# vfmatzkin/ct-unet

Hardware: AMD Instinct MI355X
Metric: voxels/sec fwd+bwd, 128^3 fp32 patch (higher is better)
Workload: dtype f32; 1 GPU; UNet() default (1 in, 2 out, i_size 8, 4 blocks), 128^3 patch, batch 1 per GPU, train step = fwd + Dice/CE loss + bwd + grad all-reduce + Adam(amsgrad); patch=128, per_gpu_batch=1, parallelism=dp1, launch=hipgraph

## Files before the change

### ct-unet_amd/csrc/conv3d.hip

```cpp
#include "common.h"
#include "pack.h"
#include "bn_tail.h"

#ifndef CTU_K3S_OCC
#define CTU_K3S_OCC 2
#endif
#ifndef CTU_K3S_ALL
#define CTU_K3S_ALL 1
#endif
#ifndef CTU_WG_OCC
#define CTU_WG_OCC 2
#endif
#ifndef CTU_WG_BLOCKS
#define CTU_WG_BLOCKS 512
#endif

namespace {

typedef float gv2f __attribute__((ext_vector_type(2)));

struct ConvP {
    const float* in;
    const float* in_scale;
    const float* in_shift;
// ... 1056 lines not shown
    const bool a_ok = (ci0 + quad * 4) < p.cin_p, g_ok = (co0 + quad * 4) < p.cout_p;
    const bool has_xf = p.in_scale != nullptr;
    float4 sc = make_float4(1.f, 1.f, 1.f, 1.f), sh = make_float4(0.f, 0.f, 0.f, 0.f);
    if (has_xf && a_ok) {
        sc = *reinterpret_cast<const float4*>(p.in_scale + ci0 + quad * 4);
        sh = *reinterpret_cast<const float4*>(p.in_shift + ci0 + quad * 4);
    }

    for (int tile = blockIdx.x; tile < p.ntiles; tile += gridDim.x) {
        int bx = tile;
        const int tx = bx % p.tiles_w; bx /= p.tiles_w;
        const int ty = bx % p.tiles_h; bx /= p.tiles_h;
        const int tz = bx % p.tiles_d; bx /= p.tiles_d;
        const int n_img = bx;
        const int d0 = tz * TD, h0 = ty * TH, w0 = tx * TW;
        __syncthreads();
        constexpr int SB = 8;
        const size_t img = (size_t)n_img * p.D * p.H * p.W;
        for (int it0 = tid; it0 < HV * 4; it0 += SB * 256) {
            f32x4 vv[SB];
            unsigned okm = 0;
#pragma unroll
            for (int q = 0; q < SB; ++q) {
                const int it = it0 + q * 256;
                const int v = (it < HV * 4 ? it : it0) >> 2;
                const int pw = v % HW, t2 = v / HW, ph = t2 % HH, pd = t2 / HH;
                const int gd = d0 + pd + kd0 - PAD, gh = h0 + ph - PAD, gw = w0 + pw - PAD;
                const bool ok = a_ok && (unsigned)gd < (unsigned)p.D && (unsigned)gh < (unsigned)p.H && (unsigned)gw < (unsigned)p.W;
                okm |= ok ? (1u << q) : 0u;
                const size_t off = ok ? ((size_t)(gd * p.H + gh) * p.W + gw) * p.in_cs + ci0 + quad * 4 : (size_t)0;
                vv[q] = *reinterpret_cast<const f32x4*>(p.in + img * p.in_cs + off);
            }
#pragma unroll
            for (int q = 0; q < SB; ++q) {
                const int it = it0 + q * 256;
                if (it < HV * 4) {
                    float4 val = make_float4(vv[q][0], vv[q][1], vv[q][2], vv[q][3]);
                    if (has_xf) val = xform4(val, sc, sh, p.in_relu);
                    if (!((okm >> q) & 1u)) val = make_float4(0.f, 0.f, 0.f, 0.f);
                    *reinterpret_cast<float4*>(&sA[(it >> 2) * 16 + quad * 4]) = val;
                }
            }
        }
        for (int it0 = tid; it0 < NVOX * 4; it0 += SB * 256) {
            f32x4 vv[SB];
            unsigned okm = 0;
#pragma unroll
            for (int q = 0; q < SB; ++q) {
                const int it = it0 + q * 256;
                const int v = (it < NVOX * 4 ? it : it0) >> 2;
                const int tw = v % TW, th = (v / TW) % TH, td = v / (TW * TH);
                const int gd = d0 + td, gh = h0 + th, gw = w0 + tw;
                const bool ok = g_ok && gd < p.D && gh < p.H && gw < p.W;
                okm |= ok ? (1u << q) : 0u;
                const size_t off = ok ? ((size_t)(gd * p.H + gh) * p.W + gw) * p.g_cs + co0 + quad * 4 : (size_t)0;
                vv[q] = *reinterpret_cast<const f32x4*>(p.g + img * p.g_cs + off);
            }
#pragma unroll
            for (int q = 0; q < SB; ++q) {
                const int it = it0 + q * 256;
                if (it < NVOX * 4)
                    *reinterpret_cast<f32x4*>(&sG[(it >> 2) * 16 + quad * 4]) = ((okm >> q) & 1u) ? vv[q] : f32x4{0.f, 0.f, 0.f, 0.f};
            }
        }
        __syncthreads();
#pragma unroll 2
        for (int ks = 0; ks < KPW; ++ks) {
            const int vt = (wave * KPW + ks) * 4 + kq;
            const int tw = vt % TW, th = (vt / TW) % TH, td = vt / (TW * TH);
            const float b = sG[vt * 16 + i];
            const int ab = ((td * HH + th) * HW + tw) * 16 + i;
#pragma unroll
            for (int t = 0; t < BT; ++t) {
                const int kd = t / (KS * KS), kh = (t / KS) % KS, kw = t % KS;
                const float a = sA[ab + ((kd * HH + kh) * HW + kw) * 16];
                acc[t] = __builtin_amdgcn_mfma_f32_16x16x4f32(a, b, acc[t], 0, 0, 0);
            }
        }
    }
    constexpr int RT = (HV * 16 / 1024) < 8 ? (HV * 16 / 1024) : 8;
    static_assert(RT >= 1 && 4 * RT * 256 <= HV * 16, "reduction scratch must fit in sA");
    const size_t slab = (size_t)(blockIdx.z * gridDim.y + blockIdx.y) * gridDim.x + blockIdx.x;
    float* dst = p.ws + slab * (BT * 256);
    for (int t0 = 0; t0 < BT; t0 += RT) {
        __syncthreads();
#pragma unroll
        for (int t = 0; t < BT; ++t)
            if (t >= t0 && t < t0 + RT) {
#pragma unroll
                for (int r = 0; r < 4; ++r) sA[(wave * RT + (t - t0)) * 256 + (kq * 4 + r) * 16 + i] = acc[t][r];
            }
        __syncthreads();
        const int nt = (BT - t0) < RT ? (BT - t0) : RT;
        for (int e = tid; e < nt * 256; e += 256)
            dst[t0 * 256 + e] = (sA[e] + sA[RT * 256 + e]) + (sA[2 * RT * 256 + e] + sA[3 * RT * 256 + e]);
    }
}

template <int KS, int KDS>
__global__ __launch_bounds__(1024) void conv3d_wgrad_reduce_kernel(const float* __restrict__ ws, float* __restrict__ dw,
                                                                  int Co, int Ci, const int32_t* __restrict__ pmap,
                                                                  int cin_p, int n_ci_t, int gx) {
    constexpr int TAPS = KS * KS * KS, BT = KDS * KS * KS;
    __shared__ float red[RPARTS][64];
    const int e = threadIdx.x & 63, part = threadIdx.x >> 6;
    const int el = blockIdx.x * 64 + e;
    const int pz = blockIdx.y;
    float s = 0.f;
    if (el < BT * 256) {
        const float* src = ws + (size_t)pz * gx * (BT * 256) + el;
        for (int k = part; k < gx; k += RPARTS) s += src[(size_t)k * (BT * 256)];
    }
    red[part][e] = s;
    __syncthreads();
    if (part == 0 && el < BT * 256) {
        const float tot = red_total(red, e);
        const int n_pairs = gridDim.y / (TAPS / BT);
        const int z = pz / n_pairs, pair = pz % n_pairs;
        const int cit = pair % n_ci_t, cot = pair / n_ci_t;
        const int tl = el >> 8, i = (el >> 4) & 15, j = el & 15;
        const int cip = cit * 16 + i, co = cot * 16 + j;
        const int ci = (cip < cin_p) ? (pmap ? pmap[cip] : (cip < Ci ? cip : -1)) : -1;
        if (ci >= 0 && co < Co) dw[((size_t)co * Ci + ci) * TAPS + z * BT + tl] = tot;
    }
}

inline bool use_k3s(int k, int W, int cin_p, int cout_p) { return k == 3 && W >= 16 && (CTU_K3S_ALL || cin_p == 8 || cout_p == 8); }

inline int wgrad_gx(int ntiles, int pairs_z) {
    int gx = CTU_WG_BLOCKS / pairs_z;
    if (gx < 1) gx = 1;
    if (gx > ntiles) gx = ntiles;
    return gx;
}


template <int SM, int SN, int UP = 0, bool LZ = false>
__global__ __launch_bounds__(256, CTU_K3S_OCC) void conv3d_wgrad_k3s_kernel(WgP p, int tiles_per_block) {
    static_assert(!UP || (SM == 1 && SN == 1), "the fused up-convolution uses the full 16 x 16 channel tile");
    constexpr int TD = 4, TH = 4, TW = (SM == 2 && SN == 2) ? 16 : 8, HD = 6, HH = 6, HW = TW + 2, HV = HD * HH * HW;
    constexpr int KPR = TW / 4, NKS = TH * KPR;
    constexpr int CM = 16 / SM, CN = 16 / SN;
    constexpr int GW = TW + (SN - 1), GV = TD * TH * GW;
    constexpr int QN = (SM == 2 && SN == 2) ? 1 : ((SM == 1 && SN == 1) ? 3 : 2);
    constexpr int NMF = UP == 2 ? 12 : (UP ? 8 : 9 * QN);
    constexpr int AQ = CM / 4, GQ = CN / 4;
    constexpr int AITEMS = HV * AQ, AITER = (AITEMS + 255) / 256;
    constexpr int GITEMS = GV * GQ, GITER = (GITEMS + 255) / 256;

    constexpr int SAF = AITER * 256 * 4, SGF = GITER * 256 * 4;
    static_assert(SAF >= HV * CM && SGF >= GV * CN, "stage size");
    __shared__ __attribute__((aligned(16))) float sA[2 * SAF];
    __shared__ __attribute__((aligned(16))) float sG[2 * SGF];

    const int tid = threadIdx.x, lane = tid & 63, wave = tid >> 6;
    const int i = lane & 15, kq = lane >> 4;
    const int cig = blockIdx.y % p.n_ci_t, cog = UP ? (blockIdx.y / p.n_ci_t) % p.n_co_t : blockIdx.y / p.n_ci_t;
    const int par = UP ? blockIdx.y / (p.n_ci_t * p.n_co_t) : 0;
    const int pz = UP == 2 ? (par >> 1) & 1 : (par >> 2) & 1, py = UP == 2 ? par & 1 : (par >> 1) & 1, px = UP == 2 ? 0 : par & 1;
    const int gH = UP ? 2 * p.H : p.H, gW = UP ? 2 * p.W : p.W, gs = UP ? 2 : 1;
    const int ci0 = cig * CM, co0 = cog * CN;
    const bool has_xf = p.in_scale != nullptr;

    f32x4 acc[NMF];
#pragma unroll
    for (int t = 0; t < NMF; ++t) acc[t] = f32x4{0.f, 0.f, 0.f, 0.f};

    const int aq = tid % AQ, gq = tid % GQ;
    const bool a_ok = (ci0 + aq * 4) < p.cin_p, g_ok = (co0 + gq * 4) < p.cout_p;
    float4 sc = make_float4(1.f, 1.f, 1.f, 1.f), sh = make_float4(0.f, 0.f, 0.f, 0.f);
    if (has_xf && a_ok) {
        sc = *reinterpret_cast<const float4*>(p.in_scale + ci0 + aq * 4);
        sh = *reinterpret_cast<const float4*>(p.in_shift + ci0 + aq * 4);
    }
    const int xf_relu = has_xf ? p.in_relu : 0;
    const int boff = (SN == 2) ? ((i < 8) ? i : i - 16) : i;

    int tile = blockIdx.x * tiles_per_block;
    const int tile_end = min(p.ntiles, tile + tiles_per_block);
    float4 va[AITER], vg[GITER];
    float4 vy[LZ ? GITER : 1];
    float4 l_sc = make_float4(0.f, 0.f, 0.f, 0.f), l_sh = l_sc, l_k0 = l_sc, l_A = l_sc, l_B = l_sc;
    if constexpr (LZ) {
        const int lzc = (co0 + ((UP && !g_ok) ? 0 : gq * 4)) % p.lz_cp;
        l_sc = *reinterpret_cast<const float4*>(p.lz_scale + lzc);
        l_sh = *reinterpret_cast<const float4*>(p.lz_shift + lzc);
        l_k0 = *reinterpret_cast<const float4*>(p.lz_coef + lzc);
        l_A = *reinterpret_cast<const float4*>(p.lz_coef + 3 * p.lz_cp + lzc);
        l_B = *reinterpret_cast<const float4*>(p.lz_coef + 4 * p.lz_cp + lzc);
    }
    const long long lz_ydelta = LZ ? reinterpret_cast<const char*>(p.lz_y) - reinterpret_cast<const char*>(p.g) : 0;
    const long long lz_odelta = LZ ? reinterpret_cast<const char*>(p.lz_out) - reinterpret_cast<const char*>(p.g) : 0;

    unsigned aoff[AITER], goff[GITER];
    constexpr int FPW = 5;
    unsigned fw[(AITER + FPW - 1) / FPW], gw0 = 0;
#pragma unroll
    for (int q = 0; q < (AITER + FPW - 1) / FPW; ++q) fw[q] = 0;
#pragma unroll
    for (int it = 0; it < AITER; ++it) {
        const int e = tid + it * 256, v = (e < AITEMS) ? e / AQ : 0;
        const int pw = v % HW, t2 = v / HW, ph = t2 % HH, pd = t2 / HH;
        aoff[it] = (unsigned)(((pd * p.H + ph) * p.W + pw) * p.in_cs + ci0 + aq * 4) * 4u;
        const unsigned face = (pd == 0 ? 1u : 0u) | (pd == HD - 1 ? 2u : 0u) | (ph == 0 ? 4u : 0u) | (ph == HH - 1 ? 8u : 0u) |
                              (pw == 0 ? 16u : 0u) | (pw == HW - 1 ? 32u : 0u);
        fw[it / FPW] |= face << (6 * (it % FPW));
    }
#pragma unroll
    for (int it = 0; it < GITER; ++it) {
        const int e = tid + it * 256, v = (e < GITEMS) ? e / GQ : 0;
        const int tw = v % GW, th = (v / GW) % TH, td = v / (GW * TH);
        goff[it] = (unsigned)(((gs * td * gH + gs * th) * gW + gs * tw) * p.g_cs + co0 + gq * 4) * 4u;
        if (SN == 2 && tw == 0) gw0 |= 1u << it;
    }
    const unsigned safe_a = (unsigned)(((p.H + 1) * p.W + 1) * p.in_cs + ci0 + ((UP && !a_ok) ? 0 : aq * 4)) * 4u;
    const unsigned safe_g = (unsigned)((SN - 1) * p.g_cs + co0 + ((UP && !g_ok) ? 0 : gq * 4)) * 4u;
    const bool ch_full = UP || (ci0 + CM <= p.cin_p && co0 + CN <= p.cout_p);

    struct Box { int tx, ty, tz, n; };
    Box box;
    {
        int t = tile;
        box.tx = t % p.tiles_w; t /= p.tiles_w;
        box.ty = t % p.tiles_h; t /= p.tiles_h;
        box.tz = t % p.tiles_d; box.n = t / p.tiles_d;
    }
    auto box_next = [&](Box b) {
        if (++b.tx == p.tiles_w) { b.tx = 0; if (++b.ty == p.tiles_h) { b.ty = 0; if (++b.tz == p.tiles_d) { b.tz = 0; ++b.n; } } }
        return b;
    };

    unsigned amask = 0, gmask = 0;
    const char* pf_abase = nullptr;
    const char* pf_gbase = nullptr;
    unsigned pf_bface = 0;
    auto prep = [&](Box b) -> bool {
        const int d0 = b.tz * TD, h0 = b.ty * TH, w0 = b.tx * TW;
        const long long org = (((long long)b.n * p.D + d0) * p.H + h0) * p.W + w0;
        pf_abase = reinterpret_cast<const char*>(p.in + (org - ((long long)p.H * p.W + p.W + 1)) * p.in_cs);
        if (UP) {
            const long long gorg = (((long long)b.n * 2 * p.D + 2 * d0 + pz) * gH + 2 * h0 + py) * gW + 2 * w0 + px;
            pf_gbase = reinterpret_cast<const char*>(p.g + gorg * p.g_cs);
        } else {
            pf_gbase = reinterpret_cast<const char*>(p.g + (org - (SN - 1)) * p.g_cs);
        }
        pf_bface = (d0 == 0 ? 1u : 0u) | (d0 + TD == p.D ? 2u : 0u) | (h0 == 0 ? 4u : 0u) | (h0 + TH == p.H ? 8u : 0u) |
                   (w0 == 0 ? 16u : 0u) | (w0 + TW == p.W ? 32u : 0u);
        amask = 0; gmask = 0;
        return ch_full && d0 + TD <= p.D && h0 + TH <= p.H && w0 + TW <= p.W;
    };
    auto fetch_a = [&](int it) {
        const bool ok = (fw[it / FPW] & (pf_bface << (6 * (it % FPW)))) == 0u && (!UP || a_ok);
        va[it] = *reinterpret_cast<const float4*>(pf_abase + (ok ? aoff[it] : safe_a));
        amask |= ok ? (1u << it) : 0u;
    };
    auto fetch_g = [&](int it) {
        const bool ok = !((pf_bface & 16u) && ((gw0 >> it) & 1u)) && (!UP || g_ok);
        const unsigned off = ok ? goff[it] : safe_g;
        vg[it] = *reinterpret_cast<const float4*>(pf_gbase + off);
        if constexpr (LZ) vy[it] = *reinterpret_cast<const float4*>(pf_gbase + lz_ydelta + off);
        gmask |= ok ? (1u << it) : 0u;
    };
    auto load_ragged = [&](Box b) {
        const int d0 = b.tz * TD, h0 = b.ty * TH, w0 = b.tx * TW;
#pragma unroll
        for (int it = 0; it < AITER; ++it) {
            const int e = tid + it * 256, v = e / AQ;
            const int pw = v % HW, t2 = v / HW, ph = t2 % HH, pd = t2 / HH;
            const int gd = d0 + pd - 1, gh = h0 + ph - 1, gw = w0 + pw - 1;
            const bool ok = e < AITEMS && a_ok && (unsigned)gd < (unsigned)p.D && (unsigned)gh < (unsigned)p.H &&
                            (unsigned)gw < (unsigned)p.W;
            float4 val = make_float4(0.f, 0.f, 0.f, 0.f);
            if (ok) {
                val = *reinterpret_cast<const float4*>(pf_abase + aoff[it]);
                amask |= 1u << it;
            }
            va[it] = val;
        }
#pragma unroll
        for (int it = 0; it < GITER; ++it) {
            const int e = tid + it * 256, v = e / GQ;
            const int tw = v % GW, th = (v / GW) % TH, td = v / (GW * TH);
            const int gd = d0 + td, gh = h0 + th, gw = w0 + tw - (SN - 1);
            const bool ok = e < GITEMS && g_ok && gd < p.D && gh < p.H && (unsigned)gw < (unsigned)p.W;
            float4 val = make_float4(0.f, 0.f, 0.f, 0.f);
            if (ok) {
                val = *reinterpret_cast<const float4*>(pf_gbase + goff[it]);
                gmask |= 1u << it;
            }
            vg[it] = val;
        }
    };

    typedef const volatile __attribute__((address_space(3))) float* lds_f_ptr;
    lds_f_ptr vA = (lds_f_ptr)sA + (((wave + pz) * HH + py) * HW + kq + px) * CM + i;
    lds_f_ptr vG = (lds_f_ptr)sG + ((wave * TH * GW + kq + (SN - 1)) * CN + boff);

    auto put_a = [&](int it, int st) {
        const float4 t = xform4(va[it], sc, sh, xf_relu);
        const bool ok = (amask >> it) & 1u;
        *reinterpret_cast<float4*>(&sA[st * SAF + (tid + it * 256) * 4]) =
            make_float4(ok ? t.x : 0.f, ok ? t.y : 0.f, ok ? t.z : 0.f, ok ? t.w : 0.f);
    };
    auto put_g = [&](int it, int st) {
        const bool ok = (gmask >> it) & 1u;
        float4 t = vg[it];
        if constexpr (LZ) {
            t = bn_bwd_lazy4(vg[it], vy[it], l_sc, l_sh, l_k0, l_A, l_B);
            *reinterpret_cast<float4*>(const_cast<char*>(pf_gbase) + lz_odelta + (ok ? goff[it] : safe_g)) = t;
        }
        *reinterpret_cast<float4*>(&sG[st * SGF + (tid + it * 256) * 4]) =
            make_float4(ok ? t.x : 0.f, ok ? t.y : 0.f, ok ? t.z : 0.f, ok ? t.w : 0.f);
    };

    constexpr bool INLOOP_FETCH = (SM == 2 && SN == 2);
    int cur = 0;
    auto stage = [&](auto fetch_tag) {
        constexpr bool FETCH = decltype(fetch_tag)::value;
        constexpr int R = 12, NJ = NKS * NMF;
        constexpr int KW0 = NKS / 2, NIT = AITER + GITER;
        constexpr int IPF = (NIT + KW0 - 1) / KW0;
        lds_f_ptr cA = vA + cur * SAF;
        lds_f_ptr cG = vG + cur * SGF;
        float ar[R], br[2];
        auto a_read = [&](int j) -> float {
            const int ks = j / NMF, t = j % NMF;
            const int th = ks / KPR, tw4 = (ks % KPR) * 4;
            const int r = UP == 2 ? t / 3 : (UP ? (t >> 1) : t / QN), q = UP == 2 ? t % 3 : (UP ? (t & 1) : t % QN),
                      kd = UP ? (r >> 1) : r / 3, kh = UP ? (r & 1) : r % 3;
            return cA[((kd * HH + th + kh) * HW + tw4 + q) * CM];
        };
        auto b_read = [&](int ks) -> float { return cG[((ks / KPR) * GW + (ks % KPR) * 4) * CN]; };
        br[0] = b_read(0);
#pragma unroll
        for (int j = 0; j < R; ++j) ar[j] = a_read(j);
        static_assert(R == 12, "fake-use list");
        asm volatile("" : "+v"(ar[0]), "+v"(ar[1]), "+v"(ar[2]), "+v"(ar[3]), "+v"(ar[4]), "+v"(ar[5]), "+v"(ar[6]),
                     "+v"(ar[7]), "+v"(ar[8]), "+v"(ar[9]), "+v"(ar[10]), "+v"(ar[11]), "+v"(br[0]));
#pragma unroll
        for (int ks = 0; ks < NKS; ++ks) {
            if (ks + 1 < NKS) {
                br[(ks + 1) & 1] = b_read(ks + 1);
                __builtin_amdgcn_sched_group_barrier(0x100, 1, 0);
            }
#pragma unroll
            for (int t = 0; t < NMF; ++t) {
                const int j = ks * NMF + t;
                acc[t] = __builtin_amdgcn_mfma_f32_16x16x4f32(ar[j % R], br[ks & 1], acc[t], 0, 0, 0);
                if (j + R < NJ) ar[j % R] = a_read(j + R);
                __builtin_amdgcn_sched_group_barrier(0x008, 1, 0);
                if (j + R < NJ) __builtin_amdgcn_sched_group_barrier(0x100, 1, 0);
#if CTU_PIN_VALU
                if (ks >= KW0) __builtin_amdgcn_sched_group_barrier(0x002, CTU_PIN_VALU, 0);
#endif
            }
            if (FETCH && ks < KW0) {
#pragma unroll
                for (int q = 0; q < IPF; ++q) {
                    const int it = ks * IPF + q;
                    if (it < AITER) fetch_a(it);
                    else if (it < NIT) fetch_g(it - AITER);
                }
            }
            if (ks >= KW0) {
                constexpr int NK2 = NKS - KW0;
#pragma unroll
                for (int it = (ks - KW0) * NIT / NK2; it < (ks - KW0 + 1) * NIT / NK2; ++it) {
                    if (it < GITER) put_g(it, cur ^ 1);
                    else put_a(it - GITER, cur ^ 1);
                }
            }
            __builtin_amdgcn_sched_barrier(0);
        }
    };

    if (tile < tile_end) {
        if (prep(box)) {
#pragma unroll
            for (int it = 0; it < AITER; ++it) fetch_a(it);
#pragma unroll
            for (int it = 0; it < GITER; ++it) fetch_g(it);
        } else {
            load_ragged(box);
        }
#pragma unroll
        for (int it = 0; it < AITER; ++it) put_a(it, 0);
#pragma unroll
        for (int it = 0; it < GITER; ++it) put_g(it, 0);
    }
    __syncthreads();
    while (tile < tile_end) {
        box = box_next(box);
        bool full = false;
        if (tile + 1 < tile_end) {
            full = prep(box);
            if (!full) load_ragged(box);
        }
        if (INLOOP_FETCH && full) {
            stage(std::true_type{});
        } else {
            if (INLOOP_FETCH == false && full) {
#pragma unroll
                for (int it = 0; it < AITER; ++it) fetch_a(it);
#pragma unroll
                for (int it = 0; it < GITER; ++it) fetch_g(it);
            }
            stage(std::false_type{});
        }
        __syncthreads();
        cur ^= 1;
        ++tile;
    }
    constexpr int RT = (2 * SAF / 1024) < NMF ? (2 * SAF / 1024) : NMF;
    static_assert(RT >= 1, "reduction scratch");
    const size_t slab = (size_t)blockIdx.y * gridDim.x + blockIdx.x;
    float* dst = p.ws + slab * (NMF * 256);
    for (int t0 = 0; t0 < NMF; t0 += RT) {
        __syncthreads();
#pragma unroll
        for (int t = 0; t < NMF; ++t)
            if (t >= t0 && t < t0 + RT) {
#pragma unroll
                for (int r = 0; r < 4; ++r) sA[(wave * RT + (t - t0)) * 256 + (kq * 4 + r) * 16 + i] = acc[t][r];
            }
        __syncthreads();
        const int nt = (NMF - t0) < RT ? (NMF - t0) : RT;
        for (int e = tid; e < nt * 256; e += 256)
            dst[t0 * 256 + e] = (sA[e] + sA[RT * 256 + e]) + (sA[2 * RT * 256 + e] + sA[3 * RT * 256 + e]);
    }
}

template <int SM, int SN>
__global__ __launch_bounds__(1024) void conv3d_wgrad_k3s_reduce_kernel(const float* __restrict__ ws, float* __restrict__ dw,
                                                                      int Co, int Ci, const int32_t* __restrict__ cinv,
                                                                      int cin_p, int n_ci_g, int gx) {
    constexpr int QN = (SM == 2 && SN == 2) ? 1 : ((SM == 1 && SN == 1) ? 3 : 2);
    constexpr int NMF = 9 * QN;
    constexpr int CM = 16 / SM, CN = 16 / SN;
    __shared__ float red[RPARTS][64];
    const int e = threadIdx.x & 63, part = threadIdx.x >> 6;
    const int el = blockIdx.x * 64 + e;
    const int pair = blockIdx.y;
    float s = 0.f;
    if (el < NMF * 256) {
        const float* src = ws + (size_t)pair * gx * (NMF * 256) + el;
        for (int k = part; k < gx; k += RPARTS) s += src[(size_t)k * (NMF * 256)];
    }
    red[part][e] = s;
    __syncthreads();
    if (part != 0 || el >= NMF * 256) return;
    const float tot = red_total(red, e);
    const int t = el >> 8, i = (el >> 4) & 15, j = el & 15;
    const int r = t / QN, q = t % QN;
    const int sm = (SM == 2) ? i / 8 : 0, cil = (SM == 2) ? i % 8 : i;
    const int sn = (SN == 2) ? j / 8 : 0, col = (SN == 2) ? j % 8 : j;
    int kw;
    bool ok = true;
    if (SM == 1 && SN == 1) kw = q;
    else if (SM == 2 && SN == 2) { kw = sm + sn; ok = !(sm == 0 && sn == 1); }
    else if (SN == 2) { if (q == 0) { kw = 0; ok = sn == 0; } else kw = 1 + sn; }
    else { if (q == 0) kw = sm; else { kw = 2; ok = sm == 1; } }
    const int cig = pair % n_ci_g, cog = pair / n_ci_g;
    const int cip = cig * CM + cil, co = cog * CN + col;
    const int ci = (cip < cin_p) ? (cinv ? cinv[cip] : (cip < Ci ? cip : -1)) : -1;
    if (ok && ci >= 0 && co < Co) dw[((size_t)co * Ci + ci) * 27 + r * 3 + kw] = tot;
}

static bool k3s_lazy_ok(int D, int H, int W, int k, int cin_p, int cout_p) {
    if (!use_k3s(k, W, cin_p, cout_p)) return false;
    const int sm = cin_p == 8 ? 2 : 1, sn = cout_p == 8 ? 2 : 1, tw = (sm == 2 && sn == 2) ? 16 : 8;
    return D % 4 == 0 && H % 4 == 0 && W % tw == 0 && cin_p % (16 / sm) == 0 && cout_p % (16 / sn) == 0;
}

template <int SM, int SN>
__global__ __launch_bounds__(256, 2) void conv3d_wgrad_k5s_kernel(WgP p, int tiles_per_block) {
    constexpr int UP = 0, PAD = 2;
    const int kd = blockIdx.z;
    constexpr int TD = 4, TH = 4, TW = (SM == 2 && SN == 2) ? 16 : 8, HD = TD, HH = TH + 2 * PAD, HW = TW + 2 * PAD, HV = HD * HH * HW;
    constexpr int KPR = TW / 4, NKS = TH * KPR;
    constexpr int CM = 16 / SM, CN = 16 / SN;
    constexpr int GW = TW + (SN - 1), GV = TD * TH * GW;
    constexpr int QN = (SM == 2 && SN == 2) ? 2 : ((SM == 1 && SN == 1) ? 5 : (SN == 2 ? 4 : 3));
    constexpr int NMF = 5 * QN;
    constexpr int AQ = CM / 4, GQ = CN / 4;
    constexpr int AITEMS = HV * AQ, AITER = (AITEMS + 255) / 256;
    constexpr int GITEMS = GV * GQ, GITER = (GITEMS + 255) / 256;

    constexpr int SAF = AITER * 256 * 4, SGF = GITER * 256 * 4;
    static_assert(SAF >= HV * CM && SGF >= GV * CN, "stage size");
    __shared__ __attribute__((aligned(16))) float sA[2 * SAF];
    __shared__ __attribute__((aligned(16))) float sG[2 * SGF];

    const int tid = threadIdx.x, lane = tid & 63, wave = tid >> 6;
    const int i = lane & 15, kq = lane >> 4;
    const int cig = blockIdx.y % p.n_ci_t, cog = UP ? (blockIdx.y / p.n_ci_t) % p.n_co_t : blockIdx.y / p.n_ci_t;
    const int par = UP ? blockIdx.y / (p.n_ci_t * p.n_co_t) : 0;
    const int pz = UP == 2 ? (par >> 1) & 1 : (par >> 2) & 1, py = UP == 2 ? par & 1 : (par >> 1) & 1, px = UP == 2 ? 0 : par & 1;
    const int gH = UP ? 2 * p.H : p.H, gW = UP ? 2 * p.W : p.W, gs = UP ? 2 : 1;
    const int ci0 = cig * CM, co0 = cog * CN;
    const bool has_xf = p.in_scale != nullptr;

    f32x4 acc[NMF];
#pragma unroll
    for (int t = 0; t < NMF; ++t) acc[t] = f32x4{0.f, 0.f, 0.f, 0.f};

    const int aq = tid % AQ, gq = tid % GQ;
    const bool a_ok = (ci0 + aq * 4) < p.cin_p, g_ok = (co0 + gq * 4) < p.cout_p;
    float4 sc = make_float4(1.f, 1.f, 1.f, 1.f), sh = make_float4(0.f, 0.f, 0.f, 0.f);
    if (has_xf && a_ok) {
        sc = *reinterpret_cast<const float4*>(p.in_scale + ci0 + aq * 4);
        sh = *reinterpret_cast<const float4*>(p.in_shift + ci0 + aq * 4);
    }
    const int xf_relu = has_xf ? p.in_relu : 0;
    const int boff = (SN == 2) ? ((i < 8) ? i : i - 16) : i;

    int tile = blockIdx.x * tiles_per_block;
    const int tile_end = min(p.ntiles, tile + tiles_per_block);
    float4 va[AITER], vg[GITER];

    unsigned aoff[AITER], goff[GITER];
    constexpr int FPW = 5;
    unsigned fw[(AITER + FPW - 1) / FPW], gw0 = 0;
#pragma unroll
    for (int q = 0; q < (AITER + FPW - 1) / FPW; ++q) fw[q] = 0;
#pragma unroll
    for (int it = 0; it < AITER; ++it) {
        const int e = tid + it * 256, v = (e < AITEMS) ? e / AQ : 0;
        const int pw = v % HW, t2 = v / HW, ph = t2 % HH, pd = t2 / HH;
        aoff[it] = (unsigned)((((pd + kd) * p.H + ph) * p.W + pw) * p.in_cs + ci0 + aq * 4) * 4u;
        const unsigned face = (pd + kd < PAD ? 1u : 0u) | (pd + kd >= TD + PAD ? 2u : 0u) | (ph < PAD ? 4u : 0u) |
                              (ph >= HH - PAD ? 8u : 0u) | (pw < PAD ? 16u : 0u) | (pw >= HW - PAD ? 32u : 0u);
        fw[it / FPW] |= face << (6 * (it % FPW));
    }
#pragma unroll
    for (int it = 0; it < GITER; ++it) {
        const int e = tid + it * 256, v = (e < GITEMS) ? e / GQ : 0;
        const int tw = v % GW, th = (v / GW) % TH, td = v / (GW * TH);
        goff[it] = (unsigned)(((gs * td * gH + gs * th) * gW + gs * tw) * p.g_cs + co0 + gq * 4) * 4u;
        if (SN == 2 && tw == 0) gw0 |= 1u << it;
    }
    const unsigned safe_a = (unsigned)(((PAD * p.H + PAD) * p.W + PAD) * p.in_cs + ci0 + aq * 4) * 4u;
    const unsigned safe_g = (unsigned)((SN - 1) * p.g_cs + co0 + ((UP && !g_ok) ? 0 : gq * 4)) * 4u;
    const bool ch_full = UP || (ci0 + CM <= p.cin_p && co0 + CN <= p.cout_p);

    struct Box { int tx, ty, tz, n; };
    Box box;
    {
        int t = tile;
        box.tx = t % p.tiles_w; t /= p.tiles_w;
        box.ty = t % p.tiles_h; t /= p.tiles_h;
        box.tz = t % p.tiles_d; box.n = t / p.tiles_d;
    }
    auto box_next = [&](Box b) {
        if (++b.tx == p.tiles_w) { b.tx = 0; if (++b.ty == p.tiles_h) { b.ty = 0; if (++b.tz == p.tiles_d) { b.tz = 0; ++b.n; } } }
        return b;
    };

    unsigned amask = 0, gmask = 0;
    const char* pf_abase = nullptr;
    const char* pf_gbase = nullptr;
    unsigned pf_bface = 0;
    auto prep = [&](Box b) -> bool {
        const int d0 = b.tz * TD, h0 = b.ty * TH, w0 = b.tx * TW;
        const long long org = (((long long)b.n * p.D + d0) * p.H + h0) * p.W + w0;
        pf_abase = reinterpret_cast<const char*>(p.in + (org - (long long)PAD * ((long long)p.H * p.W + p.W + 1)) * p.in_cs);
        if (UP) {
            const long long gorg = (((long long)b.n * 2 * p.D + 2 * d0 + pz) * gH + 2 * h0 + py) * gW + 2 * w0 + px;
            pf_gbase = reinterpret_cast<const char*>(p.g + gorg * p.g_cs);
        } else {
            pf_gbase = reinterpret_cast<const char*>(p.g + (org - (SN - 1)) * p.g_cs);
        }
        pf_bface = (d0 == 0 ? 1u : 0u) | (d0 + TD == p.D ? 2u : 0u) | (h0 == 0 ? 4u : 0u) | (h0 + TH == p.H ? 8u : 0u) |
                   (w0 == 0 ? 16u : 0u) | (w0 + TW == p.W ? 32u : 0u);
        amask = 0; gmask = 0;
        return ch_full && d0 + TD <= p.D && h0 + TH <= p.H && w0 + TW <= p.W && (d0 + TD == p.D || d0 + TD + PAD <= p.D) &&
               (h0 + TH == p.H || h0 + TH + PAD <= p.H) && (w0 + TW == p.W || w0 + TW + PAD <= p.W);
    };
    auto fetch_a = [&](int it) {
        const bool ok = (fw[it / FPW] & (pf_bface << (6 * (it % FPW)))) == 0u && (!UP || a_ok);
        va[it] = *reinterpret_cast<const float4*>(pf_abase + (ok ? aoff[it] : safe_a));
        amask |= ok ? (1u << it) : 0u;
    };
    auto fetch_g = [&](int it) {
        const bool ok = !((pf_bface & 16u) && ((gw0 >> it) & 1u)) && (!UP || g_ok);
        vg[it] = *reinterpret_cast<const float4*>(pf_gbase + (ok ? goff[it] : safe_g));
        gmask |= ok ? (1u << it) : 0u;
    };
    auto load_ragged = [&](Box b) {
        const int d0 = b.tz * TD, h0 = b.ty * TH, w0 = b.tx * TW;
#pragma unroll
        for (int it = 0; it < AITER; ++it) {
            const int e = tid + it * 256, v = e / AQ;
            const int pw = v % HW, t2 = v / HW, ph = t2 % HH, pd = t2 / HH;
            const int gd = d0 + pd + kd - PAD, gh = h0 + ph - PAD, gw = w0 + pw - PAD;
            const bool ok = e < AITEMS && a_ok && (unsigned)gd < (unsigned)p.D && (unsigned)gh < (unsigned)p.H &&
                            (unsigned)gw < (unsigned)p.W;
            float4 val = make_float4(0.f, 0.f, 0.f, 0.f);
            if (ok) {
                val = *reinterpret_cast<const float4*>(pf_abase + aoff[it]);
                amask |= 1u << it;
            }
            va[it] = val;
        }
#pragma unroll
        for (int it = 0; it < GITER; ++it) {
            const int e = tid + it * 256, v = e / GQ;
            const int tw = v % GW, th = (v / GW) % TH, td = v / (GW * TH);
            const int gd = d0 + td, gh = h0 + th, gw = w0 + tw - (SN - 1);
            const bool ok = e < GITEMS && g_ok && gd < p.D && gh < p.H && (unsigned)gw < (unsigned)p.W;
            float4 val = make_float4(0.f, 0.f, 0.f, 0.f);
            if (ok) {
                val = *reinterpret_cast<const float4*>(pf_gbase + goff[it]);
                gmask |= 1u << it;
            }
            vg[it] = val;
        }
    };

    typedef const volatile __attribute__((address_space(3))) float* lds_f_ptr;
    lds_f_ptr vA = (lds_f_ptr)sA + (((wave + pz) * HH + py) * HW + kq + px) * CM + i;
    lds_f_ptr vG = (lds_f_ptr)sG + ((wave * TH * GW + kq + (SN - 1)) * CN + boff);

    auto put_a = [&](int it, int st) {
        const float4 t = xform4(va[it], sc, sh, xf_relu);
        const bool ok = (amask >> it) & 1u;
        *reinterpret_cast<float4*>(&sA[st * SAF + (tid + it * 256) * 4]) =
            make_float4(ok ? t.x : 0.f, ok ? t.y : 0.f, ok ? t.z : 0.f, ok ? t.w : 0.f);
    };
    auto put_g = [&](int it, int st) {
        const bool ok = (gmask >> it) & 1u;
        *reinterpret_cast<float4*>(&sG[st * SGF + (tid + it * 256) * 4]) =
            make_float4(ok ? vg[it].x : 0.f, ok ? vg[it].y : 0.f, ok ? vg[it].z : 0.f, ok ? vg[it].w : 0.f);
    };

    constexpr bool INLOOP_FETCH = (SM == 2 && SN == 2);
    int cur = 0;
    auto stage = [&](auto fetch_tag) {
        constexpr bool FETCH = decltype(fetch_tag)::value;
        constexpr int R = 12, NJ = NKS * NMF;
        constexpr int KW0 = NKS / 2, NIT = AITER + GITER;
        constexpr int IPF = (NIT + KW0 - 1) / KW0;
        lds_f_ptr cA = vA + cur * SAF;
        lds_f_ptr cG = vG + cur * SGF;
        float ar[R], br[2];
        auto a_read = [&](int j) -> float {
            const int ks = j / NMF, t = j % NMF;
            const int th = ks / KPR, tw4 = (ks % KPR) * 4;
            const int kh = t / QN, q = t % QN;
            const int t0 = (SM == 1) ? q : ((SN == 1 && q == 2) ? 3 : 2 * q);
            return cA[((th + kh) * HW + tw4 + t0) * CM];
        };
        auto b_read = [&](int ks) -> float { return cG[((ks / KPR) * GW + (ks % KPR) * 4) * CN]; };
        br[0] = b_read(0);
#pragma unroll
        for (int j = 0; j < R; ++j) ar[j] = a_read(j);
        static_assert(R == 12, "fake-use list");
        asm volatile("" : "+v"(ar[0]), "+v"(ar[1]), "+v"(ar[2]), "+v"(ar[3]), "+v"(ar[4]), "+v"(ar[5]), "+v"(ar[6]),
                     "+v"(ar[7]), "+v"(ar[8]), "+v"(ar[9]), "+v"(ar[10]), "+v"(ar[11]), "+v"(br[0]));
#pragma unroll
        for (int ks = 0; ks < NKS; ++ks) {
            if (ks + 1 < NKS) {
                br[(ks + 1) & 1] = b_read(ks + 1);
                __builtin_amdgcn_sched_group_barrier(0x100, 1, 0);
            }
#pragma unroll
            for (int t = 0; t < NMF; ++t) {
                const int j = ks * NMF + t;
                acc[t] = __builtin_amdgcn_mfma_f32_16x16x4f32(ar[j % R], br[ks & 1], acc[t], 0, 0, 0);
                if (j + R < NJ) ar[j % R] = a_read(j + R);
                __builtin_amdgcn_sched_group_barrier(0x008, 1, 0);
                if (j + R < NJ) __builtin_amdgcn_sched_group_barrier(0x100, 1, 0);
#if CTU_PIN_VALU
                if (ks >= KW0) __builtin_amdgcn_sched_group_barrier(0x002, CTU_PIN_VALU, 0);
#endif
            }
            if (FETCH && ks < KW0) {
#pragma unroll
                for (int q = 0; q < IPF; ++q) {
                    const int it = ks * IPF + q;
                    if (it < AITER) fetch_a(it);
                    else if (it < NIT) fetch_g(it - AITER);
                }
            }
            if (ks >= KW0) {
                constexpr int NK2 = NKS - KW0;
#pragma unroll
                for (int it = (ks - KW0) * NIT / NK2; it < (ks - KW0 + 1) * NIT / NK2; ++it) {
                    if (it < GITER) put_g(it, cur ^ 1);
                    else put_a(it - GITER, cur ^ 1);
                }
            }
            __builtin_amdgcn_sched_barrier(0);
        }
    };

    if (tile < tile_end) {
        if (prep(box)) {
#pragma unroll
            for (int it = 0; it < AITER; ++it) fetch_a(it);
#pragma unroll
            for (int it = 0; it < GITER; ++it) fetch_g(it);
        } else {
            load_ragged(box);
        }
#pragma unroll
        for (int it = 0; it < AITER; ++it) put_a(it, 0);
#pragma unroll
        for (int it = 0; it < GITER; ++it) put_g(it, 0);
    }
    __syncthreads();
    while (tile < tile_end) {
        box = box_next(box);
        bool full = false;
        if (tile + 1 < tile_end) {
            full = prep(box);
            if (!full) load_ragged(box);
        }
        if (INLOOP_FETCH && full) {
            stage(std::true_type{});
        } else {
            if (INLOOP_FETCH == false && full) {
#pragma unroll
                for (int it = 0; it < AITER; ++it) fetch_a(it);
#pragma unroll
                for (int it = 0; it < GITER; ++it) fetch_g(it);
            }
            stage(std::false_type{});
        }
        __syncthreads();
        cur ^= 1;
        ++tile;
    }
// ... 517 lines not shown
```

Baseline: 658.6 million voxels/s.

## Restructure lazy-BN wgrad kernel: single delta store, in-loop G-first fetch, vectorized reduction

In the lazy BN-backward path with UP==1, the global write-back of the recomputed gradient delta now happens only from the cig==0 block instead of every input-channel group. The same path now issues the next tile's loads inside the MFMA loop, fetching G before A. For the SM=SN=1 lazy case, the cross-wave reduction moves to f32x4 LDS stores and reads, with one wave per tile slice. Optional CTU_STAMP timing instrumentation is added; it compiles out by default.

```diff
diff --git a/ct-unet_amd/csrc/conv3d.hip b/ct-unet_amd/csrc/conv3d.hip
--- a/ct-unet_amd/csrc/conv3d.hip
+++ b/ct-unet_amd/csrc/conv3d.hip
@@ -1382,19 +1382,25 @@
         *reinterpret_cast<float4*>(&sA[st * SAF + (tid + it * 256) * 4]) =
             make_float4(ok ? t.x : 0.f, ok ? t.y : 0.f, ok ? t.z : 0.f, ok ? t.w : 0.f);
     };
+    constexpr bool LZ_STORE_ONCE = LZ && UP == 1;
+    const bool lz_store = !LZ_STORE_ONCE || cig == 0;
     auto put_g = [&](int it, int st) {
         const bool ok = (gmask >> it) & 1u;
         float4 t = vg[it];
         if constexpr (LZ) {
             t = bn_bwd_lazy4(vg[it], vy[it], l_sc, l_sh, l_k0, l_A, l_B);
-            *reinterpret_cast<float4*>(const_cast<char*>(pf_gbase) + lz_odelta + (ok ? goff[it] : safe_g)) = t;
+            if (lz_store) *reinterpret_cast<float4*>(const_cast<char*>(pf_gbase) + lz_odelta + (ok ? goff[it] : safe_g)) = t;
         }
         *reinterpret_cast<float4*>(&sG[st * SGF + (tid + it * 256) * 4]) =
             make_float4(ok ? t.x : 0.f, ok ? t.y : 0.f, ok ? t.z : 0.f, ok ? t.w : 0.f);
     };
 
-    constexpr bool INLOOP_FETCH = (SM == 2 && SN == 2);
+    constexpr bool INLOOP_FETCH = (SM == 2 && SN == 2) || (LZ && UP == 1);
+    constexpr bool G_FIRST = LZ && UP == 1;
     int cur = 0;
+#ifdef CTU_STAMP
+    unsigned long long tq0 = 0, tq1 = 0, tq2 = 0, tq3 = 0, ph[3] = {0, 0, 0}, nst = 0;
+#endif
     auto stage = [&](auto fetch_tag) {
         constexpr bool FETCH = decltype(fetch_tag)::value;
         constexpr int R = 12, NJ = NKS * NMF;
@@ -1419,6 +1425,7 @@
                      "+v"(ar[7]), "+v"(ar[8]), "+v"(ar[9]), "+v"(ar[10]), "+v"(ar[11]), "+v"(br[0]));
 #pragma unroll
         for (int ks = 0; ks < NKS; ++ks) {
+            if (ks == KW0) STAMP(tq1);
             if (ks + 1 < NKS) {
                 br[(ks + 1) & 1] = b_read(ks + 1);
                 __builtin_amdgcn_sched_group_barrier(0x100, 1, 0);
@@ -1438,8 +1445,13 @@
 #pragma unroll
                 for (int q = 0; q < IPF; ++q) {
                     const int it = ks * IPF + q;
-                    if (it < AITER) fetch_a(it);
-                    else if (it < NIT) fetch_g(it - AITER);
+                    if (G_FIRST) {
+                        if (it < GITER) fetch_g(it);
+                        else if (it < NIT) fetch_a(it - GITER);
+                    } else {
+                        if (it < AITER) fetch_a(it);
+                        else if (it < NIT) fetch_g(it - AITER);
+                    }
                 }
             }
             if (ks >= KW0) {
@@ -1470,6 +1482,7 @@
     }
     __syncthreads();
     while (tile < tile_end) {
+        STAMP(tq0);
         box = box_next(box);
         bool full = false;
         if (tile + 1 < tile_end) {
@@ -1487,27 +1500,64 @@
             }
             stage(std::false_type{});
         }
+        STAMP(tq2);
         __syncthreads();
+        STAMP(tq3);
+#ifdef CTU_STAMP
+        ph[0] += tq1 - tq0; ph[1] += tq2 - tq1; ph[2] += tq3 - tq2; ++nst;
+#endif
         cur ^= 1;
         ++tile;
     }
+    STAMP(tq0);
     constexpr int RT = (2 * SAF / 1024) < NMF ? (2 * SAF / 1024) : NMF;
     static_assert(RT >= 1, "reduction scratch");
     const size_t slab = (size_t)blockIdx.y * gridDim.x + blockIdx.x;
     float* dst = p.ws + slab * (NMF * 256);
-    for (int t0 = 0; t0 < NMF; t0 += RT) {
-        __syncthreads();
-#pragma unroll
-        for (int t = 0; t < NMF; ++t)
-            if (t >= t0 && t < t0 + RT) {
-#pragma unroll
-                for (int r = 0; r < 4; ++r) sA[(wave * RT + (t - t0)) * 256 + (kq * 4 + r) * 16 + i] = acc[t][r];
-            }
-        __syncthreads();
-        const int nt = (NMF - t0) < RT ? (NMF - t0) : RT;
-        for (int e = tid; e < nt * 256; e += 256)
-            dst[t0 * 256 + e] = (sA[e] + sA[RT * 256 + e]) + (sA[2 * RT * 256 + e] + sA[3 * RT * 256 + e]);
-    }
+    constexpr bool QUAD = LZ && SM == 1 && SN == 1 && UP != 2;
+    if constexpr (QUAD) {
+        f32x4* s4 = reinterpret_cast<f32x4*>(sA);
+#pragma unroll
+        for (int rd = 0; rd < (NMF + RT - 1) / RT; ++rd) {
+            __syncthreads();
+#pragma unroll
+            for (int tt = 0; tt < RT; ++tt)
+                if (rd * RT + tt < NMF) s4[(wave * RT + tt) * 64 + lane] = acc[rd * RT + tt];
+            __syncthreads();
+#pragma unroll
+            for (int tt0 = 0; tt0 < RT; tt0 += 4) {
+                const int tt = tt0 + wave;
+                if (tt < RT && rd * RT + tt < NMF) {
+                    const f32x4 s = (s4[tt * 64 + lane] + s4[(RT + tt) * 64 + lane]) + (s4[(2 * RT + tt) * 64 + lane] + s4[(3 * RT + tt) * 64 + lane]);
+                    float* d = dst + (rd * RT + tt) * 256 + kq * 64 + i;
+#pragma unroll
+                    for (int r = 0; r < 4; ++r) d[r * 16] = s[r];
+                }
+            }
+        }
+    } else {
+        for (int t0 = 0; t0 < NMF; t0 += RT) {
+            __syncthreads();
+#pragma unroll
+            for (int t = 0; t < NMF; ++t)
+                if (t >= t0 && t < t0 + RT) {
+#pragma unroll
+                    for (int r = 0; r < 4; ++r) sA[(wave * RT + (t - t0)) * 256 + (kq * 4 + r) * 16 + i] = acc[t][r];
+                }
+            __syncthreads();
+            const int nt = (NMF - t0) < RT ? (NMF - t0) : RT;
+            for (int e = tid; e < nt * 256; e += 256)
+                dst[t0 * 256 + e] = (sA[e] + sA[RT * 256 + e]) + (sA[2 * RT * 256 + e] + sA[3 * RT * 256 + e]);
+        }
+    }
+#ifdef CTU_STAMP
+    STAMP(tq1);
+    if (g_stamp_out && tid == 0) {
+        unsigned long long* o = g_stamp_out + slab * 6;
+        for (int k = 0; k < 3; ++k) o[k] = ph[k];
+        o[3] = tq1 - tq0; o[4] = 0; o[5] = nst;
+    }
+#endif
 }
 
 template <int SM, int SN>
```

Measured after the change: 661.4 million voxels/s (median of 6 runs). No clear change (+0.4%).
